# penincillin/IHMR

Measured on AMD Instinct MI355X. Metric: images/sec, IHMR-OPT 200-iter refinement batch=64 (ms/refine-iter: latency.ms_per_refine_iter; amortised: ms_per_refine_iter_amortised), higher is better.
Workload: dtype f32

## Files before the change

### ihmr_amd/csrc/ihmr_hip.hip

```cpp
#include <math.h>
#include <stdio.h>
#include <stdlib.h>
#include <string.h>

#include <algorithm>
#include <atomic>
#include <mutex>
#include <vector>

#include "ihmr_common.h"
#include "mano_lbs.h"
#include "sdf_collision.h"
#include "preprocess.h"
#include "augment.h"
#include "render.h"
#include "mlp_infer.h"
#include "refine.h"
#include "encoder.h"
#include "encoder_bf16.h"
#include "evaluate.h"
#include "train.h"
#include "train_conv.h"
#include "copy_pack.h"
#include "launch_plan.h"
// ... 111 lines not shown
        for (int k = 0; k < 3; ++k) {
            const int32_t id = h->faces[(f < NF ? f : 0) * 3 + k];
            if (id < 0 || id >= NV) { delete m; return -1; }
            fsoa[(size_t)k * NFP + f] = id;
        }
    std::vector<uint32_t> fpk(NFP, 0u);
    for (int f = 0; f < NFP; ++f)
        fpk[f] = (uint32_t)fsoa[f] | ((uint32_t)fsoa[(size_t)NFP + f] << 10) | ((uint32_t)fsoa[(size_t)2 * NFP + f] << 20);
    std::vector<float> pd4, sd4, vt4;
    pack4(pd.data(), NPF, pd4);
    pack4(sd_t.data(), 10, sd4);
    pack4(vt.data(), 1, vt4);
    int rc = 0;
    rc |= upload_as(&m->pd4, pd4); rc |= upload_as(&m->sd4, sd4); rc |= upload_as(&m->vt4, vt4);
    rc |= upload(&m->v_template, vt); rc |= upload(&m->shapedirs_t, sd_t); rc |= upload(&m->posedirs, pd);
    rc |= upload(&m->J_template, J_t); rc |= upload(&m->J_shapedirs, J_sd); rc |= upload(&m->weights, wts);
    rc |= upload_as(&m->w4_w, w4w); rc |= upload(&m->w4_j, w4j);
    m->sparse4 = sparse4;
    rc |= upload(&m->pose_mean, pm); rc |= upload(&m->parents, par); rc |= upload(&m->depth, depth);
    rc |= upload(&m->tip_ids, tips); rc |= upload(&m->wj_start, start); rc |= upload(&m->wj_vert, wv);
    rc |= upload(&m->wj_w, ww); rc |= upload(&m->seg_q, seg_q); rc |= upload(&m->jseg_start, jseg); rc |= upload(&m->faces, fsoa); rc |= upload(&m->faces_pk, fpk); rc |= upload(&m->J_regressor, jr);
    m->max_depth = maxd;
    m->nnz = (int)wv.size();
    m->nseg = (int)seg_q.size() - 1;
    if (m->nseg > LBS_SEG_CAP) { ihmr_mano_destroy(m); return -1; }
    {
        const int dyn = m->nseg * 12 * (int)sizeof(float);
        hipError_t e1 = hipFuncSetAttribute((const void*)lbs_bwd1_kernel<true>, hipFuncAttributeMaxDynamicSharedMemorySize, dyn);
        hipError_t e2 = hipFuncSetAttribute((const void*)lbs_bwd1_kernel<false>, hipFuncAttributeMaxDynamicSharedMemorySize, dyn);
        if (e1 != hipSuccess || e2 != hipSuccess) { ihmr_mano_destroy(m); return (int)(e1 != hipSuccess ? e1 : e2); }
        int dev = 0, lds_max = 0;
        (void)hipGetDevice(&dev);
        (void)hipDeviceGetAttribute(&lds_max, hipDeviceAttributeMaxSharedMemoryPerBlock, dev);
        const void* tails[3] = {(const void*)opt_tail_kernel<true, true>, (const void*)opt_tail_kernel<true>, (const void*)opt_tail_kernel<false>};
        m->tail_fits = 1;
        const int tail_dyn = opt_tail_dynamic_lds(m->nseg);
        for (const void* k : tails) {
            hipFuncAttributes fa;
            if (hipFuncGetAttributes(&fa, k) != hipSuccess || (long)fa.sharedSizeBytes + tail_dyn > (long)lds_max ||
                hipFuncSetAttribute(k, hipFuncAttributeMaxDynamicSharedMemorySize, tail_dyn) != hipSuccess)
                m->tail_fits = 0;
        }
        (void)hipGetLastError();
    }
    if (rc) return rc;
    *out = m;
    return 0;
}

extern "C" int ihmr_mano_destroy(ihmr_mano* m) {
    if (!m) return 0;
    void* ptrs[] = {m->v_template, m->shapedirs_t, m->posedirs, m->J_template, m->J_shapedirs, m->weights, m->pose_mean,
                    m->parents, m->depth, m->tip_ids, m->wj_start, m->wj_vert, m->wj_w, m->faces, m->J_regressor, m->pd4, m->sd4, m->vt4, m->seg_q, m->jseg_start,
                    m->w4_w, m->w4_j, m->faces_pk};
    for (void* p : ptrs)
        if (p) (void)hipFree(p);
    delete m;
    return 0;
}

extern "C" int ihmr_mano_update_shapedirs(ihmr_mano* m, const float* shapedirs_host) {
    if (!m || !shapedirs_host) return -1;
    std::vector<float> jr((size_t)NJ * NV), vt(NV3), sd_t, J_t, J_sd;
    HIP_TRY(hipMemcpy(jr.data(), m->J_regressor, jr.size() * 4, hipMemcpyDeviceToHost));
    HIP_TRY(hipMemcpy(vt.data(), m->v_template, vt.size() * 4, hipMemcpyDeviceToHost));
    derive_shape_constants(jr.data(), vt.data(), shapedirs_host, sd_t, J_t, J_sd);
    HIP_TRY(hipMemcpy(m->shapedirs_t, sd_t.data(), sd_t.size() * 4, hipMemcpyHostToDevice));
    HIP_TRY(hipMemcpy(m->J_shapedirs, J_sd.data(), J_sd.size() * 4, hipMemcpyHostToDevice));
    std::vector<float> sd4;
    pack4(sd_t.data(), 10, sd4);
    HIP_TRY(hipMemcpy(m->sd4, sd4.data(), sd4.size() * 4, hipMemcpyHostToDevice));
    return 0;
}

extern "C" size_t ihmr_mano_workspace_bytes(int N) { return lbs_ws_bytes(N); }

template <bool TWO_HAND, int MODE>
static void lbs_skin_launch_mode(const ihmr_mano* m, int N, int B, float* verts, float* joints, const LbsWork& wk, float* pose_off, hipStream_t st) {
    const bool small = N <= LBS_SMALL_MAX_HANDS;
    const int hg8 = 8 * (small ? LBS_HG_SMALL : LBS_HG);
    const dim3 skin_grid(8, 4 * ((N + hg8 - 1) / hg8));
    if (small) hipLaunchKernelGGL((lbs_skin_kernel<TWO_HAND, MODE, LBS_HG_SMALL>), skin_grid, dim3(LBS_THREADS), 0, st, *m, (const float*)wk.skel, N, B,
                                  verts, joints, wk.v_posed, pose_off);
    else hipLaunchKernelGGL((lbs_skin_kernel<TWO_HAND, MODE, LBS_HG>), skin_grid, dim3(LBS_THREADS), 0, st, *m, (const float*)wk.skel, N, B, verts,
                            joints, wk.v_posed, pose_off);
}
#define LBS_SKIN_FULL 0
#define LBS_SKIN_REUSE 1
#define LBS_SKIN_KEEP_P 2
#define LBS_SKIN_FULL_STORE_P 3
static int g_force_full_skin = 0;
template <bool TWO_HAND>
static void lbs_skin_launch(const ihmr_mano* m, int mode, int N, int B, float* verts, float* joints, const LbsWork& wk, hipStream_t st) {
    if (g_force_full_skin && (mode == LBS_SKIN_KEEP_P || mode == LBS_SKIN_FULL_STORE_P)) mode = LBS_SKIN_FULL;
    if (mode == LBS_SKIN_REUSE) lbs_skin_launch_mode<TWO_HAND, LBS_MODE_REUSE>(m, N, B, verts, joints, wk, nullptr, st);
    else if (mode == LBS_SKIN_KEEP_P) lbs_skin_launch_mode<TWO_HAND, LBS_MODE_KEEP_P>(m, N, B, verts, joints, wk, wk.pose_off, st);
    else lbs_skin_launch_mode<TWO_HAND, LBS_MODE_FULL>(m, N, B, verts, joints, wk, mode == LBS_SKIN_FULL_STORE_P ? wk.pose_off : nullptr, st);
}
extern "C" int ihmr_debug_force_full_skin(int force) {
    const int prev = g_force_full_skin;
    g_force_full_skin = force ? 1 : 0;
    return prev;
}

static void lbs_forward_launch(const ihmr_mano* m, bool two_hand, const float* orient, const float* pose, const float* betas,
                               const float* trans, int N, int B, float* verts, float* joints, const LbsWork& wk, hipStream_t st) {
    if (two_hand) {
        hipLaunchKernelGGL(lbs_skel_kernel<true>, dim3(N), dim3(192), 0, st, *m, orient, pose, betas, trans, B, wk.skel, joints);
        lbs_skin_launch<true>(m, LBS_SKIN_FULL, N, B, verts, joints, wk, st);
    } else {
        hipLaunchKernelGGL(lbs_skel_kernel<false>, dim3(N), dim3(192), 0, st, *m, orient, pose, betas, trans, B, wk.skel, joints);
        lbs_skin_launch<false>(m, LBS_SKIN_FULL, N, B, verts, joints, wk, st);
    }
}

static int g_bwd2_streaming = 0;
extern "C" int ihmr_debug_force_lbs_bwd2_streaming(int force) {
    const int prev = g_bwd2_streaming;
    g_bwd2_streaming = force ? 1 : 0;
    return prev;
}

static void lbs_backward_launch(const ihmr_mano* m, bool two_hand, int N, int B, const float* d_verts, const float* d_joints,
                                float* d_orient, float* d_pose, float* d_betas, float* d_trans, int need_mask, const LbsWork& wk,
                                hipStream_t st, bool bwd1_done = false) {
    const size_t part_lds = (size_t)m->nseg * 12 * sizeof(float);
    if (bwd1_done) {}
    else if (two_hand)
        hipLaunchKernelGGL(lbs_bwd1_kernel<true>, dim3(N), dim3(LBS_THREADS), part_lds, st, *m, wk, B, d_verts, d_joints, d_orient,
                           d_betas, d_trans, need_mask);
    else
        hipLaunchKernelGGL(lbs_bwd1_kernel<false>, dim3(N), dim3(LBS_THREADS), part_lds, st, *m, wk, B, d_verts, d_joints, d_orient,
                           d_betas, d_trans, need_mask);
    if (need_mask & 2) {
// ... 166 lines not shown
extern "C" int ihmr_opt_forward_losses(const ihmr_mano* m, const ihmr_mano* m_left, const ihmr_opt_io* io, int B,
                                       const ihmr_opt_weights* w, void* stream) {
    if (!m || !io || !w || B <= 0 || 2 * B > SDF_MAX_HANDS) return -1;
    hipStream_t st = (hipStream_t)stream;
    OptWork wk = opt_carve(io->workspace, B);
    int rc = opt_forward(m, m_left, io, wk, B, *w, kNoStep, st);
    if (rc) return rc;
    return (int)hipGetLastError();
}

extern "C" int ihmr_opt_run_stage(const ihmr_mano* m, const ihmr_mano* m_left, const ihmr_opt_io* io, int B,
                                  const ihmr_opt_weights* w, const ihmr_opt_stage* sg, void* stream) {
    if (!m || !io || !w || !sg || B <= 0 || 2 * B > SDF_MAX_HANDS || sg->n_iters <= 0 || sg->save_freq <= 0) return -1;
    if (sg->param_mask <= 0 || sg->param_mask > 255 || sg->select_loss < 0 || sg->select_loss > 2) return -1;
    if (sg->optimizer != IHMR_OPTIM_ADAM && sg->optimizer != IHMR_OPTIM_SGD) return -1;
    hipStream_t st = (hipStream_t)stream;
    OptWork wk = opt_carve(io->workspace, B);
    const int pm = sg->param_mask;
    const int need_mask = ((pm & (IHMR_PB_ORIENT_R | IHMR_PB_ORIENT_L)) ? 1 : 0) | ((pm & (IHMR_PB_POSE_R | IHMR_PB_POSE_L)) ? 2 : 0) |
                          ((pm & (IHMR_PB_SHAPE_R | IHMR_PB_SHAPE_L)) ? 4 : 0) | ((pm & IHMR_PB_TRANS) ? 8 : 0);
    const int need_cam = (pm & IHMR_PB_CAM) ? 1 : 0, sgd = sg->optimizer == IHMR_OPTIM_SGD;
    int S = 0;
    ParamStep step{0, 0.f, 0.f, 1.f, -1, 1, 0};
    const bool vposed_fixed = (pm & (IHMR_PB_POSE_R | IHMR_PB_POSE_L | IHMR_PB_SHAPE_R | IHMR_PB_SHAPE_L)) == 0;
    const bool pose_fixed = (pm & (IHMR_PB_POSE_R | IHMR_PB_POSE_L)) == 0;
    const int keep_mode = vposed_fixed ? LBS_SKIN_REUSE : (pose_fixed ? LBS_SKIN_KEEP_P : LBS_SKIN_FULL);
    const int first_mode = (!vposed_fixed && pose_fixed) ? LBS_SKIN_FULL_STORE_P : LBS_SKIN_FULL;
    const bool fused_tail = need_mask != 0 && !io->no_fused_tail && m->tail_fits;
    int static_mask = ((pm & (IHMR_PB_ORIENT_R | IHMR_PB_POSE_R | IHMR_PB_SHAPE_R)) ? 0 : 1) |
                      ((pm & (IHMR_PB_ORIENT_L | IHMR_PB_POSE_L | IHMR_PB_SHAPE_L | IHMR_PB_TRANS | IHMR_PB_SHAPE_R)) ? 0 : 2);
    if ((pm & IHMR_PB_TRANS) && !(pm & (IHMR_PB_ORIENT_L | IHMR_PB_POSE_L | IHMR_PB_SHAPE_L | IHMR_PB_SHAPE_R)) && io->sdf_no_static_reuse == 0)
        static_mask |= 2 | (2 << 2);
    const bool pose_stage = (need_mask & 2) != 0;
    const size_t tail_lds = (size_t)opt_tail_dynamic_lds(m->nseg);
    const int lists_first = sg->keep_lists ? 3 : 2;
    for (int it = 0; it < sg->n_iters; ++it) {
        const double t = (double)(it + 1);
        const double bc1 = 1.0 - pow(0.9, t), bc2 = 1.0 - pow(0.999, t);
        const ParamStep next{pm, w->shape_reg, sgd ? sg->lr : (float)((double)sg->lr / bc1), (float)sqrt(bc2),
                             (it % sg->save_freq == 0) ? S++ : -1, 0, sgd};
        if (fused_tail) {
            int rc = opt_forward(m, m_left, io, wk, B, *w, step, st, need_cam, it == 0 ? first_mode : (vposed_fixed ? -1 : keep_mode), it == 0 ? lists_first : 1,
                                 it == 0 || pose_stage, false, static_mask);
            if (rc) return rc;
            SdfWorkspace ws = opt_sdf_ws(io, wk, B, it == 0 ? lists_first : 1, static_mask);
            VertLayout vl{io->verts, (long)NV3, (long)B * NV3};
            hipEvent_t tcur;
            const bool timed = g_timer != nullptr;
            if (timed) { if (int rc2 = timed_begin(&tcur, st)) return rc2; }
            const TailArgs ta{*m, *io, wk, B, *w, vl, ws, need_cam, need_mask, next, ws.inside_count};
            if (vposed_fixed && it + 1 < sg->n_iters)
                hipLaunchKernelGGL((opt_tail_kernel<true, true>), dim3(B), dim3(SDF_SAMPLE_THREADS), tail_lds, st, ta);
            else if (!pose_stage && it + 1 < sg->n_iters)
                hipLaunchKernelGGL(opt_tail_kernel<true>, dim3(B), dim3(SDF_SAMPLE_THREADS), tail_lds, st, ta);
            else
                hipLaunchKernelGGL(opt_tail_kernel<false>, dim3(B), dim3(SDF_SAMPLE_THREADS), tail_lds, st, ta);
            if (timed) { if (int rc2 = timed_next(&tcur, IHMR_TIMED_OPT_TAIL, st)) return rc2; (void)hipEventDestroy(tcur); }
            if (pose_stage)
                lbs_backward_launch(m, true, 2 * B, B, wk.g_verts, wk.g_joints, wk.g_orient, wk.g_pose, wk.g_shape, wk.g_trans, need_mask,
                                    wk.lbs, st, true);
        } else {
            int rc = opt_forward(m, m_left, io, wk, B, *w, step, st, need_cam, it == 0 ? first_mode : keep_mode, it == 0 ? lists_first : 1, true, true, static_mask);
            if (rc) return rc;
            if (need_mask)
                lbs_backward_launch(m, true, 2 * B, B, wk.g_verts, wk.g_joints, wk.g_orient, wk.g_pose, wk.g_shape, wk.g_trans, need_mask,
                                    wk.lbs, st);
        }
        step = next;
    }
    hipLaunchKernelGGL(opt_adam_kernel, dim3(B), dim3(128), 0, st, *io, wk, B, step);
    hipLaunchKernelGGL(opt_select_kernel, dim3((B + 63) / 64), dim3(64), 0, st, *io, B, S, *sg);
    return (int)hipGetLastError();
}

extern "C" int ihmr_opt_set_params(const ihmr_opt_io* io, const float* final_params, int B, void* stream) {
    if (!io || !final_params || B <= 0) return -1;
    hipLaunchKernelGGL(opt_unpack_params_kernel, dim3(B), dim3(128), 0, (hipStream_t)stream, *io, final_params, B);
    return (int)hipGetLastError();
}

extern "C" size_t ihmr_mlp_workspace_bytes(int B) { return ((size_t)B * (512 + 256 + 128 + 126) * sizeof(float) + 256 + 255) & ~(size_t)255; }
static float* mlp_acc_joints(void* workspace, int B) { return (float*)((char*)workspace + 256) + (size_t)B * (512 + 256 + 128); }

static int mlp_fill_select(MlpSelect& s, const ihmr_mlp_tables* t, const ihmr_mlp_stage* stage, int mode, void* workspace) {
// ... 721 lines not shown
```

### ihmr_amd/csrc/mano_lbs.h

```cpp
#pragma once
#include "ihmr_common.h"

#define LBS_THREADS 256
#define LBS_HG 8
#define LBS_HG_SMALL 4
#define LBS_SMALL_MAX_HANDS 256
#define LBS_TILE_V 195
#define LBS_KG 25
#define LBS_KC 3
#define LBS_SEG 13
#define LBS_SEG_CAP 1024
#define LBS_CSR_CAP 4096

#define SK_R 0
#define SK_J 144
#define SK_G 192
#define SK_A 384
#define SK_PF 576
#define SK_POSE 712
#define SK_BETA 760
#define SK_SHIFT 770
#define SK_STRIDE 784

struct LbsWork {
    float* skel;
    float* v_posed;
    float* dvp;
    float* chain;
    float* dpf_part;
    float* pose_off;
};

static inline size_t lbs_ws_bytes(int N) {
    size_t n = (size_t)N * (SK_STRIDE + 3 * NV3 + 192 + LBS_KG * 136) * sizeof(float);
    return ((n + 255) & ~(size_t)255) + 6 * 256;
}

static inline LbsWork lbs_carve(void* ws, int N) {
    LbsWork w;
    char* p = (char*)ws;
    auto take = [&](size_t bytes) { char* r = p; p += (bytes + 255) & ~(size_t)255; return (float*)r; };
    w.skel = take((size_t)N * SK_STRIDE * 4);
    w.v_posed = take((size_t)N * NV3 * 4);
    w.dvp = take((size_t)N * NV3 * 4);
    w.chain = take((size_t)N * 192 * 4);
    w.dpf_part = take((size_t)LBS_KG * N * 136 * 4);
    w.pose_off = take((size_t)N * NV3 * 4);
    return w;
}

template <bool TWO_HAND>
__device__ __forceinline__ void lbs_skel_hand(const ihmr_mano& m, const float* __restrict__ orient,
                                              const float* __restrict__ pose, const float* __restrict__ betas,
                                              const float* __restrict__ trans, int B, float* __restrict__ skel,
                                              float* __restrict__ joints, float* sk, int h, int tid_in, bool active = true) {
    const bool left = TWO_HAND && h >= B;
    const int tid = active ? tid_in : (1 << 20);
    float* sR = sk + SK_R; float* sJ = sk + SK_J; float* sG = sk + SK_G; float* sA = sk + SK_A;
    const int my_depth = active ? m.depth[tid_in / 12] : -1, my_parent = active ? m.parents[tid_in / 12] : 0;
    float* sPF = sk + SK_PF; float* sPose = sk + SK_POSE; float* sBeta = sk + SK_BETA; float* sShift = sk + SK_SHIFT;
    if (tid < 48) {
        float v = tid < 3 ? orient[h * 3 + tid] : pose[h * 45 + tid - 3];
        if (left && (tid % 3) != 0) v = -v;
        sPose[tid] = v + m.pose_mean[tid];
    }
    if (tid >= 64 && tid < 74) sBeta[tid - 64] = betas[h * 10 + tid - 64];
    if (tid >= 128 && tid < 142) sk[SK_SHIFT + tid - 128] = 0.f;
    if (tid == 150) sPF[135] = 0.f;
    __syncthreads();
    if (tid < NJ) rodrigues_fwd(&sPose[3 * tid], &sR[9 * tid]);
    if (tid >= 64 && tid < 64 + 48) {
        const int e = tid - 64;
        float acc = m.J_template[e];
#pragma unroll
        for (int l = 0; l < 10; ++l) acc = __builtin_fmaf(m.J_shapedirs[e * 10 + l], sBeta[l], acc);
        sJ[e] = acc;
    }
    __syncthreads();
    if (tid < NPF) {
        const int j = 1 + tid / 9, e = tid % 9;
        sPF[tid] = sR[9 * j + e] - ((e == 0 || e == 4 || e == 8) ? 1.0f : 0.0f);
    }
    if (tid >= 160 && tid < 172) {
        const int e = tid - 160, r = e / 4, c = e % 4;
        sG[e] = c < 3 ? sR[3 * r + c] : sJ[r];
    }
    if (TWO_HAND && left && tid >= 176 && tid < 179) {
        const int k = tid - 176;
        const float* br = betas + (h - B) * 10;
        float jr = m.J_template[k];
#pragma unroll
        for (int l = 0; l < 10; ++l) jr = __builtin_fmaf(m.J_shapedirs[k * 10 + l], br[l], jr);
        const float jl = k == 0 ? -sJ[0] : sJ[k];
        sShift[k] = trans[(h - B) * 3 + k] + (jr - jl);
    }
    __syncthreads();
    for (int d = 1; d <= m.max_depth; ++d) {
        const int j = tid / 12, e = tid % 12, r = e / 4, c = e % 4;
        if (my_depth == d) {
            const int p = my_parent;
            sG[12 * j + e] = lbs_chain_elem(sG + 12 * p, sR + 9 * j, sJ + 3 * j, sJ + 3 * p, r, c);
        }
        __syncthreads();
    }
    if (active) {
        const int j = tid / 12, e = tid % 12, r = e / 4, c = e % 4;
        sA[12 * j + e] = lbs_rel_elem(sG + 12 * j, sJ + 3 * j, r, c);
    }
    __syncthreads();
    for (int i = tid; i < SK_STRIDE; i += 192) skel[(size_t)h * SK_STRIDE + i] = sk[i];
    if (tid < NJ * 3) {
        const int j = tid / 3, k = tid % 3;
// ... 881 lines not shown
```

### ihmr_amd/csrc/refine.h

```cpp
#pragma once
#include "ihmr_common.h"

#define LOSS_THREADS 64
#define OPT_NPARAM IHMR_OPT_NPARAM

struct OptWork {
    LbsWork lbs;
    float* joints_raw;
    float* g_verts;
    float* g_joints;
    float* g_trans_direct;
    float* g_cam;
    float* g_orient;
    float* g_pose;
    float* g_shape;
    float* g_trans;
    void* sdf_ws;
};

static inline size_t opt_ws_bytes(int B) {
    size_t n = 0;
    n += (size_t)2 * B * NV3 * 4;
    n += lbs_ws_bytes(2 * B);
    n += (size_t)B * 42 * 3 * 4 * 2;
    n += (size_t)B * (3 + 6 + 90 + 20 + 3 + 3 + 1) * 4;
    n = (n + 255) & ~(size_t)255;
    n += 8192;
    return n + sdf_ws_bytes(2 * B, true);
}

static inline OptWork opt_carve(void* ws, int B) {
    OptWork w;
    char* p = (char*)ws;
    auto take = [&](size_t bytes) { char* r = p; p += (bytes + 255) & ~(size_t)255; return r; };
    w.lbs = lbs_carve(take(lbs_ws_bytes(2 * B)), 2 * B);
    w.g_verts = (float*)take((size_t)2 * B * NV3 * 4);
    w.joints_raw = (float*)take((size_t)B * 42 * 3 * 4);
    w.g_joints = (float*)take((size_t)B * 42 * 3 * 4);
    w.g_trans_direct = (float*)take((size_t)B * 3 * 4);
    w.g_orient = (float*)take((size_t)B * 6 * 4);
    w.g_pose = (float*)take((size_t)B * 90 * 4);
    w.g_shape = (float*)take((size_t)B * 20 * 4);
    w.g_trans = (float*)take((size_t)B * 3 * 4);
    w.g_cam = (float*)take((size_t)B * 3 * 4);
    w.sdf_ws = (void*)p;
    return w;
}

__constant__ int c_finger_ids[20] = {1, 2, 3, 17, 4, 5, 6, 18, 7, 8, 9, 20, 10, 11, 12, 19, 13, 14, 15, 16};

struct LossShared {
    float raw[42][3], p1[42][3], p2[42][3], g2[42][3], acc[8][LOSS_THREADS], gsum[2][3];
};
#define LOSS_SYNC()                                                  \
    do {                                                             \
        __builtin_amdgcn_fence(__ATOMIC_RELEASE, "workgroup");       \
        __builtin_amdgcn_wave_barrier();                             \
        __builtin_amdgcn_fence(__ATOMIC_ACQUIRE, "workgroup");       \
    } while (0)

__device__ __forceinline__ void opt_loss_wave(const ihmr_opt_io& io, const OptWork& wk, int B, const ihmr_opt_weights& w,
                                              LossShared& sh, int b, int j, int need_cam, LbsBwdShared* gj_lds = nullptr) {
    const bool act = j < 42;
    const int Bn = io.norm_batch > 0 ? io.norm_batch : B;
    const int jj = act ? j : 0;
    const float cs = io.cam[b * 3], ctx = io.cam[b * 3 + 1], cty = io.cam[b * 3 + 2];
    float r[3], t2[3], tg2[3], tg3[4], ti3[4];
#pragma unroll
    for (int k = 0; k < 3; ++k) {
        r[k] = wk.joints_raw[(b * 42 + jj) * 3 + k];
        t2[k] = io.init_joints_2d[(b * 42 + jj) * 3 + k];
        tg2[k] = io.gt_joints_2d[(b * 42 + jj) * 3 + k];
    }
#pragma unroll
    for (int k = 0; k < 4; ++k) { tg3[k] = io.gt_joints_3d[(b * 42 + jj) * 4 + k]; ti3[k] = io.init_joints_3d[(b * 42 + jj) * 4 + k]; }
    float tp4[4] = {0.f, 0.f, 0.f, 0.f}, tgt4[4] = {0.f, 0.f, 0.f, 0.f}, tr3[3] = {0.f, 0.f, 0.f};
    if (j == 5) {
#pragma unroll
        for (int k = 0; k < 4; ++k) { tp4[k] = io.init_hand_trans_j[b * 4 + k]; tgt4[k] = io.gt_hand_trans[b * 4 + k]; }
#pragma unroll
        for (int k = 0; k < 3; ++k) tr3[k] = io.trans[b * 3 + k];
    }
    __builtin_amdgcn_sched_barrier(0);
    if (act) {
#pragma unroll
        for (int k = 0; k < 3; ++k) sh.raw[j][k] = r[k];
    }
    LOSS_SYNC();

    float l2d_p = 0.f, l2d_gt = 0.f, g_raw[3] = {0.f, 0.f, 0.f};
    if (act) {
        const float px = (r[0] + ctx) * cs, py = (r[1] + cty) * cs;
        io.joints_2d[(b * 42 + j) * 2] = px;
        io.joints_2d[(b * 42 + j) * 2 + 1] = py;
        const float dx = t2[0] - px, dy = t2[1] - py;
// ... 214 lines not shown
}
__device__ __forceinline__ void opt_snapshot_losses(const ihmr_opt_io& io, int B, const ParamStep& st, int b, int e) {
    if (st.snap_idx >= 0 && e < 3) io.snap_loss[((size_t)st.snap_idx * 3 + e) * B + b] = io.loss_batch[e * B + b];
}

__global__ __launch_bounds__(128) void opt_adam_kernel(ihmr_opt_io io, OptWork wk, int B, ParamStep st) {
    opt_snapshot_losses(io, B, st, blockIdx.x, threadIdx.x);
    if ((int)threadIdx.x < OPT_NPARAM) opt_param_apply(io, wk, B, st, blockIdx.x, threadIdx.x);
}

__global__ __launch_bounds__(384) void opt_adam_skel_kernel(ihmr_mano m, ihmr_opt_io io, OptWork wk, int B, ParamStep st,
                                                            int* inside_count) {
    TL_SCOPE(7);
    __shared__ float sk[2][SK_STRIDE];
    const int b = blockIdx.x, tid = threadIdx.x;
    if (b == 0 && tid >= 192 && tid < 192 + SDF_NZERO) sdf_zero_counter(inside_count, tid - 192);
    if (st.reset_state && tid < OPT_NPARAM) { io.adam_m[b * OPT_NPARAM + tid] = 0.f; io.adam_v[b * OPT_NPARAM + tid] = 0.f; }
    if (st.mask && tid < OPT_NPARAM) { opt_snapshot_losses(io, B, st, b, tid); opt_param_apply(io, wk, B, st, b, tid); }
    __syncthreads();
    const int hl = tid / 192;
    lbs_skel_hand<true>(m, io.orient, io.pose, io.shape, io.trans, B, wk.lbs.skel, wk.joints_raw, sk[hl], hl * B + b, tid % 192);
}

#ifdef TAIL_STAMPS
__device__ long long g_tail_stamps[3][4096][8];
#define TAIL_TK(k) do { if (threadIdx.x == 0) { const long long now_ = (long long)__builtin_readcyclecounter(); if (blockIdx.x < 4096) g_tail_stamps[STEP + SKIN][blockIdx.x][k] += now_ - tk_prev_; tk_prev_ = now_; } } while (0)
#else
#define TAIL_TK(k)
#endif
static inline int opt_tail_dynamic_lds(int nseg) { return 2 * nseg * 12 * (int)sizeof(float); }
struct TailArgs {
    ihmr_mano m; ihmr_opt_io io; OptWork wk; int B; ihmr_opt_weights w; VertLayout vl; SdfWorkspace ws; int need_cam, need_mask;
    ParamStep st; int* inside_count;
};
__device__ __forceinline__ const TailArgs& tail_args() {
    typedef const __attribute__((address_space(4))) TailArgs* ArgPtr;
    ArgPtr p = (ArgPtr)__builtin_amdgcn_kernarg_segment_ptr();
    asm volatile("" : "+s"(p));
    return *(const TailArgs*)p;
}
template <bool STEP, bool SKIN = false>
__global__ __launch_bounds__(SDF_SAMPLE_THREADS, 4) void opt_tail_kernel(TailArgs) {
    TL_SCOPE(3 + (STEP ? 1 : 0) + (SKIN ? 1 : 0));
    __shared__ LossShared sh;
    __shared__ float red16[SDF_SAMPLE_THREADS / WAVE];
    __shared__ LbsBwdShared bw[2];
    extern __shared__ __attribute__((aligned(16))) float tail_part[];
    const int b = blockIdx.x, tid = threadIdx.x;
#ifdef TAIL_STAMPS
    long long tk_prev_ = (long long)__builtin_readcyclecounter();
    if (tid == 0 && blockIdx.x < 4096) g_tail_stamps[STEP + SKIN][blockIdx.x][7] += 1;
#endif
    const int hl = tid / LBS_THREADS;
    {
    const TailArgs& a = tail_args();
    const int B = a.B, need_mask = a.need_mask;
    const ihmr_opt_io io = a.io; const OptWork wk = a.wk; const ihmr_opt_weights w = a.w; const SdfWorkspace ws = a.ws;
    const VertLayout vl = a.vl;
    if ((need_mask & 7) != 0) {
        lds_dma_dwords(wk.lbs.v_posed + (size_t)(hl * B + b) * NV3, bw[hl].vp, NV3, tid % LBS_THREADS, LBS_THREADS);
        lds_dma_dwords(wk.lbs.skel + (size_t)(hl * B + b) * SK_STRIDE, bw[hl].sk, SK_STRIDE, tid % LBS_THREADS, LBS_THREADS);
    } else if (SKIN) {
        lds_dma_dwords(wk.lbs.skel + (size_t)(hl * B + b) * SK_STRIDE, bw[hl].sk, SK_STRIDE, tid % LBS_THREADS, LBS_THREADS);
    }
    const float mask = (io.hand_type_array[b * 2] + io.hand_type_array[b * 2 + 1]) > 1.5f ? 1.f : 0.f;
    const float gs = w.collision * mask / (ws.loss_div * (float)(io.norm_batch > 0 ? io.norm_batch : B));
// ... 35 lines not shown
    uint32_t jr[VR];
    if (SKIN) {
#pragma unroll
        for (int r = 0; r < VR; ++r) {
            const int v = min(lt + r * LBS_THREADS, NV - 1);
            const float* s0 = wk.lbs.v_posed + ((size_t)hv * NV + v) * 3;
            vp[r][0] = s0[0]; vp[r][1] = s0[1]; vp[r][2] = s0[2];
            wr[r] = m.sparse4 ? m.w4_w[v] : make_float4(0.f, 0.f, 0.f, 0.f);
            jr[r] = m.sparse4 ? m.w4_j[v] : 0u;
        }
        __builtin_amdgcn_sched_barrier(0);
    }
    if (SKIN && (need_mask & 7) == 0) {
        if (tid < 3) {
            const float* br = io.shape + (size_t)b * 10;
            float jr = m.J_template[tid];
#pragma unroll
            for (int l = 0; l < 10; ++l) jr = __builtin_fmaf(m.J_shapedirs[tid * 10 + l], br[l], jr);
            const float* sJl = bw[1].sk + SK_J;
            const float jl = tid == 0 ? -sJl[0] : sJl[tid];
            const float sh = io.trans[b * 3 + tid] + (jr - jl);
            bw[1].sk[SK_SHIFT + tid] = sh;
            wk.lbs.skel[((size_t)B + b) * SK_STRIDE + SK_SHIFT + tid] = sh;
        }
        __syncthreads();
        if (tid < NJ * 3) {
            const int j = tid / 3, k = tid % 3;
            const float val = bw[1].sk[SK_G + 12 * j + 4 * k + 3];
            wk.joints_raw[((size_t)b * 42 + 21 + j) * 3 + k] = (k == 0 ? -val : val) + bw[1].sk[SK_SHIFT + k];
        }
    } else {
        const int hs = tid / 192;
        lbs_skel_hand<true>(m, io.orient, io.pose, io.shape, io.trans, B, wk.lbs.skel, wk.joints_raw, bw[hs < 2 ? hs : 0].sk, (hs < 2 ? hs : 0) * B + b, tid % 192,
                            hs < 2);
    }
    TAIL_TK(3);
    if (!SKIN) return;
    const float* sA = bw[hl].sk + SK_A;
    const float* sShift = bw[hl].sk + SK_SHIFT;
#pragma unroll
    for (int r = 0; r < VR; ++r) {
        const int v = lt + r * LBS_THREADS;
        if (v >= NV) break;
        float T[12];
#pragma unroll
        for (int e = 0; e < 12; ++e) T[e] = 0.f;
        if (m.sparse4) {
            const float wv[4] = {wr[r].x, wr[r].y, wr[r].z, wr[r].w};
#pragma unroll
            for (int sI = 0; sI < 4; ++sI) {
                const float4* A4 = reinterpret_cast<const float4*>(sA + 12 * (int)((jr[r] >> (8 * sI)) & 0xffu));
#pragma unroll
                for (int q = 0; q < 3; ++q) {
                    const float4 a = A4[q];
                    T[4 * q] = __builtin_fmaf(wv[sI], a.x, T[4 * q]);
                    T[4 * q + 1] = __builtin_fmaf(wv[sI], a.y, T[4 * q + 1]);
                    T[4 * q + 2] = __builtin_fmaf(wv[sI], a.z, T[4 * q + 2]);
                    T[4 * q + 3] = __builtin_fmaf(wv[sI], a.w, T[4 * q + 3]);
                }
            }
        } else {
            for (int j = 0; j < NJ; ++j) {
                const float wj = m.weights[v * NJ + j];
#pragma unroll
                for (int e = 0; e < 12; ++e) T[e] = __builtin_fmaf(wj, sA[12 * j + e], T[e]);
            }
        }
        float out[3];
#pragma unroll
        for (int q = 0; q < 3; ++q) out[q] = T[4 * q + 0] * vp[r][0] + T[4 * q + 1] * vp[r][1] + T[4 * q + 2] * vp[r][2] + T[4 * q + 3];
        if (hl == 1) {
            out[0] = -out[0] + sShift[0];
            out[1] = out[1] + sShift[1];
            out[2] = out[2] + sShift[2];
        }
        float* dst = io.verts + ((size_t)hv * NV + v) * 3;
        dst[0] = out[0]; dst[1] = out[1]; dst[2] = out[2];
#pragma unroll
        for (int t = 0; t < IHMR_NUM_TIPS; ++t)
            if (v == m.tip_ids[t]) {
                float* jd = wk.joints_raw + ((size_t)b * 42 + (hl ? 21 : 0) + NJ + t) * 3;
                jd[0] = out[0]; jd[1] = out[1]; jd[2] = out[2];
            }
    }
    TAIL_TK(4);
}

__global__ __launch_bounds__(256) void mlp_camera_select_kernel(ihmr_opt_io io, OptWork wk, int B, ihmr_opt_weights w, MlpSelect sel) {
    __shared__ LossShared sh;
    const int b = blockIdx.x, tid = threadIdx.x;
    if (tid < WAVE) {
        opt_loss_wave(io, wk, B, w, sh, b, tid, 0);
        if (tid == 0) io.loss_batch[(size_t)2 * B + b] = sel.prev_loss[(size_t)sel.idx[b] * 3 + 2];
    }
    mlp_select_sample(sel, io.loss_batch, B, b);
}

__global__ __launch_bounds__(128) void opt_unpack_params_kernel(ihmr_opt_io io, const float* __restrict__ packed, int B) {
    const int b = blockIdx.x, e = threadIdx.x;
    if (e >= 122) return;
    const float v = packed[(size_t)b * 122 + e];
    if (e < 3) io.cam[b * 3 + e] = v;
    else if (e < 6) io.orient[(size_t)b * 3 + (e - 3)] = v;
    else if (e < 51) io.pose[(size_t)b * 45 + (e - 6)] = v;
    else if (e < 54) io.orient[((size_t)B + b) * 3 + (e - 51)] = v;
    else if (e < 99) io.pose[((size_t)B + b) * 45 + (e - 54)] = v;
    else if (e < 109) io.shape[(size_t)b * 10 + (e - 99)] = v;
    else if (e < 119) io.shape[((size_t)B + b) * 10 + (e - 109)] = v;
    else io.trans[b * 3 + (e - 119)] = v;
}

__global__ void opt_select_kernel(ihmr_opt_io io, int B, int S, ihmr_opt_stage sg) {
    const int b = blockIdx.x * blockDim.x + threadIdx.x;
    if (b >= B) return;
    float bar[3];
#pragma unroll
    for (int l = 0; l < 3; ++l) bar[l] = io.snap_loss[(size_t)l * B + b] * sg.filter_factor[l];
    int best = 0;
// ... 16 lines not shown
```

### ihmr_amd/hip.py

```python
from __future__ import annotations

import ctypes as C
import os
import os.path as osp
import subprocess

import numpy as np
import torch

_HERE = osp.dirname(osp.abspath(__file__))
LIB_PATH = osp.join(_HERE, "libihmr_hip.so")
SRC_DIR = osp.join(_HERE, "csrc")
HIPCC_FLAGS = ["--offload-arch=gfx950", "-O3", "-std=c++17", "-ffp-contract=off", "-shared", "-fPIC"]

NUM_VERTS, NUM_FACES, NUM_JOINTS, OPT_NPARAM = 778, 1538, 16, 122
PARAM_BLOCKS = dict(pred_cam_params=(1, 0, 3), pred_hand_trans=(2, 3, 3), pred_right_orient=(4, 6, 3), pred_left_orient=(8, 9, 3),
                    pred_right_pose_params=(16, 12, 45), pred_left_pose_params=(32, 57, 45),
                    pred_right_shape_params=(64, 102, 10), pred_left_shape_params=(128, 112, 10))
LOSS_IDS = dict(joints_2d_loss_p=0, joints_3d_loss_p=1, collision_loss=2)
OPTIMIZERS = dict(adam=0, sgd=1)

EXPORTED_SYMBOLS = [
    "ihmr_mano_create", "ihmr_mano_destroy", "ihmr_mano_update_shapedirs", "ihmr_mano_workspace_bytes", "ihmr_mano_lbs_fwd",
    "ihmr_mano_lbs_bwd",
    "ihmr_sdf_workspace_bytes", "ihmr_sdf_collision", "ihmr_sdf_collision_ex", "ihmr_sdf_dense_grid", "ihmr_opt_workspace_bytes",
    "ihmr_opt_run_stage", "ihmr_opt_forward_losses", "ihmr_opt_sdf_stats", "ihmr_opt_sdf_counters", "ihmr_opt_sdf_inside_bits", "ihmr_opt_stage_graph_create",
    "ihmr_opt_forward_graph_create", "ihmr_graph_launch", "ihmr_graph_destroy", "ihmr_opt_set_params", "ihmr_eval_metrics", "ihmr_eval_mpvpe", "ihmr_conv_igemm", "ihmr_maxpool3x3s2",
    "ihmr_avgpool_relu", "ihmr_preprocess_images", "ihmr_mlp_train_grad", "ihmr_transpose", "ihmr_relu_backward", "ihmr_colsum",
    "ihmr_adam_step", "ihmr_bn_workspace_bytes", "ihmr_bn_train_forward", "ihmr_bn_train_backward", "ihmr_conv_wgrad",
    "ihmr_dilate2", "ihmr_interleave2", "ihmr_pack_dgrad_weight", "ihmr_maxpool3x3s2_backward", "ihmr_avgpool_relu_backward", "ihmr_set_kernel_timer", "ihmr_flush_kernel_timer",
    "ihmr_mlp_workspace_bytes", "ihmr_mlp_stage_head", "ihmr_mlp_forward_select", "ihmr_mlp_camera_select", "ihmr_opt_forward_verts",
    "ihmr_debug_force_lbs_bwd2_streaming", "ihmr_debug_force_full_skin", "ihmr_version", "ihmr_copy_segments", "ihmr_root_align_joints",
    "ihmr_augment_images", "ihmr_augment_labels",
    "ihmr_render_workspace_bytes", "ihmr_render_meshes", "ihmr_draw_keypoints",
    "ihmr_conv_igemm_bf16", "ihmr_pack_image_bf16", "ihmr_maxpool3x3s2_bf16", "ihmr_avgpool_relu_bf16", "ihmr_cast_f32_bf16",
]


class ManoArrays(C.Structure):
    _fields_ = [(n, C.c_void_p) for n in ("v_template", "shapedirs", "posedirs", "J_regressor", "lbs_weights", "parents",
                                          "hands_mean", "faces", "tip_ids")]


class OptIO(C.Structure):
    _fields_ = [(n, C.c_void_p) for n in (
        "cam", "trans", "orient", "pose", "shape",
        "init_joints_2d", "init_joints_3d", "init_hand_trans_j", "gt_joints_2d", "gt_joints_3d", "gt_hand_trans",
        "hand_type_array",
        "verts", "joints_3d", "joints_2d", "loss_batch", "coll_per_vert", "coll_origin_scale",
        "snap_params", "snap_loss", "selected", "adam_m", "adam_v", "workspace")] + [
        ("norm_batch", C.c_int), ("sdf_align_corners", C.c_int), ("sdf_loss_divisor", C.c_float), ("sdf_swap_xz", C.c_int),
        ("sdf_no_candidate_lists", C.c_int), ("sdf_no_static_reuse", C.c_int),
        ("no_fused_tail", C.c_int)]


class CopySeg(C.Structure):
    _fields_ = [("src", C.c_void_p), ("dst", C.c_void_p), ("rows", C.c_int), ("width", C.c_int), ("src_ld", C.c_int), ("dst_ld", C.c_int)]


COPY_MAX_SEGS = 32


def copy_segments(pairs):
    segs = []
    for src, dst in pairs:
# ... 285 lines not shown
```

### include/ihmr_hip.h

```cpp
#ifndef IHMR_HIP_H
#define IHMR_HIP_H

#include <stddef.h>
#include <stdint.h>

#ifdef __cplusplus
extern "C" {
#endif

#define IHMR_NUM_VERTS 778
#define IHMR_NUM_FACES 1538
#define IHMR_NUM_JOINTS 16
#define IHMR_NUM_TIPS 5
#define IHMR_SDF_GRID 32

typedef struct ihmr_mano_arrays {
    const float* v_template;
    const float* shapedirs;
    const float* posedirs;
    const float* J_regressor;
    const float* lbs_weights;
    const int32_t* parents;
    const float* hands_mean;
    const int32_t* faces;
// ... 195 lines not shown
int ihmr_draw_keypoints(uint8_t* img, const float* kps, const float* weight, const uint8_t* colour, int B, int S, int K, void* stream);

#define IHMR_TIMED_SDF_PREP 0
#define IHMR_TIMED_SDF_DIST 1
#define IHMR_TIMED_OPT_TAIL 2
#define IHMR_TIMED_KERNELS 4
typedef struct ihmr_kernel_timer { double ms[IHMR_TIMED_KERNELS]; long n[IHMR_TIMED_KERNELS]; double ms_event_pair; long n_event_pair; } ihmr_kernel_timer;
int ihmr_set_kernel_timer(ihmr_kernel_timer* t);
int ihmr_flush_kernel_timer(void);

typedef struct ihmr_mlp_net { const float* w[4]; const float* b[4]; int ldw[4]; int k_out; int col[122]; } ihmr_mlp_net;
typedef struct ihmr_mlp_tables {
    const int64_t* idx;
    uint8_t* data_idxs_all;
    float* img_feat_all;
    float* prev_final;
    float* prev_loss;
    const float* img_feat;
    float* new_params;
    float* final_params;
    uint8_t* kept;
} ihmr_mlp_tables;
typedef struct ihmr_mlp_stage { int n_filter; int filter_loss[4]; float filter_factor[4]; int select_loss; } ihmr_mlp_stage;
size_t ihmr_mlp_workspace_bytes(int B);
int ihmr_mlp_stage_head(const ihmr_mlp_net* net, const ihmr_mlp_tables* t, const ihmr_opt_io* io, int B, void* workspace, void* stream);
int ihmr_mlp_forward_select(const ihmr_mano* m, const ihmr_mano* m_left, const ihmr_opt_io* io, int B, const ihmr_opt_weights* w,
                            const ihmr_mlp_tables* t, const ihmr_mlp_stage* stage, int mode, void* workspace, void* stream);
int ihmr_mlp_camera_select(const ihmr_opt_io* io, int B, const ihmr_opt_weights* w, const ihmr_mlp_tables* t, const ihmr_mlp_stage* stage,
                           void* workspace, void* stream);
int ihmr_opt_forward_verts(const ihmr_mano* m, const ihmr_opt_io* io, int B, void* stream);

int ihmr_debug_force_lbs_bwd2_streaming(int force);
int ihmr_debug_force_full_skin(int force);

const char* ihmr_version(void);

#ifdef __cplusplus
}
#endif
#endif
```

Before: 29030.

## Add translation-only fused tail kernel and skip rotation recompute for fixed hands

Adds a dedicated opt_tail_kernel_trans for stages where only translation is optimized. It computes the trans gradient as a direct sum of per-vertex SDF gradients and caches the skinned left-hand vertices once, so later iterations only add the shift instead of redoing skinning. It also passes a keep_rot flag so the skeleton pass skips the Rodrigues and pose-feature recompute for hands whose orient and pose are frozen. The cost is an extra per-batch vertex buffer in the workspace and correctness that depends on the cached state staying valid across iterations.

```diff
diff --git a/ihmr_amd/csrc/ihmr_hip.hip b/ihmr_amd/csrc/ihmr_hip.hip
--- a/ihmr_amd/csrc/ihmr_hip.hip
+++ b/ihmr_amd/csrc/ihmr_hip.hip
@@ -167,13 +167,15 @@
         int dev = 0, lds_max = 0;
         (void)hipGetDevice(&dev);
         (void)hipDeviceGetAttribute(&lds_max, hipDeviceAttributeMaxSharedMemoryPerBlock, dev);
-        const void* tails[3] = {(const void*)opt_tail_kernel<true, true>, (const void*)opt_tail_kernel<true>, (const void*)opt_tail_kernel<false>};
+        const void* tails[4] = {(const void*)opt_tail_kernel<true, true>, (const void*)opt_tail_kernel<true>, (const void*)opt_tail_kernel<false>,
+                                (const void*)opt_tail_kernel_trans};
         m->tail_fits = 1;
         const int tail_dyn = opt_tail_dynamic_lds(m->nseg);
         for (const void* k : tails) {
             hipFuncAttributes fa;
-            if (hipFuncGetAttributes(&fa, k) != hipSuccess || (long)fa.sharedSizeBytes + tail_dyn > (long)lds_max ||
-                hipFuncSetAttribute(k, hipFuncAttributeMaxDynamicSharedMemorySize, tail_dyn) != hipSuccess)
+            const int dyn_k = k == (const void*)opt_tail_kernel_trans ? 0 : tail_dyn;
+            if (hipFuncGetAttributes(&fa, k) != hipSuccess || (long)fa.sharedSizeBytes + dyn_k > (long)lds_max ||
+                (dyn_k && hipFuncSetAttribute(k, hipFuncAttributeMaxDynamicSharedMemorySize, dyn_k) != hipSuccess))
                 m->tail_fits = 0;
         }
         (void)hipGetLastError();
@@ -235,6 +237,12 @@
 extern "C" int ihmr_debug_force_full_skin(int force) {
     const int prev = g_force_full_skin;
     g_force_full_skin = force ? 1 : 0;
+    return prev;
+}
+static int g_force_generic_tail = 0;
+extern "C" int ihmr_debug_force_generic_tail(int force) {
+    const int prev = g_force_generic_tail;
+    g_force_generic_tail = force ? 1 : 0;
     return prev;
 }
 
@@ -467,6 +475,9 @@
     if ((pm & IHMR_PB_TRANS) && !(pm & (IHMR_PB_ORIENT_L | IHMR_PB_POSE_L | IHMR_PB_SHAPE_L | IHMR_PB_SHAPE_R)) && io->sdf_no_static_reuse == 0)
         static_mask |= 2 | (2 << 2);
     const bool pose_stage = (need_mask & 2) != 0;
+    const bool trans_tail = vposed_fixed && need_mask == 8 && !g_force_generic_tail;
+    const int keep_rot = ((need_mask & 7) == 0 || g_force_generic_tail) ? 0
+                         : (((pm & (IHMR_PB_ORIENT_R | IHMR_PB_POSE_R)) ? 0 : 1) | ((pm & (IHMR_PB_ORIENT_L | IHMR_PB_POSE_L)) ? 0 : 2));
     const size_t tail_lds = (size_t)opt_tail_dynamic_lds(m->nseg);
     const int lists_first = sg->keep_lists ? 3 : 2;
     for (int it = 0; it < sg->n_iters; ++it) {
@@ -483,8 +494,10 @@
             hipEvent_t tcur;
             const bool timed = g_timer != nullptr;
             if (timed) { if (int rc2 = timed_begin(&tcur, st)) return rc2; }
-            const TailArgs ta{*m, *io, wk, B, *w, vl, ws, need_cam, need_mask, next, ws.inside_count};
-            if (vposed_fixed && it + 1 < sg->n_iters)
+            const TailArgs ta{*m, *io, wk, B, *w, vl, ws, need_cam, need_mask, next, ws.inside_count, keep_rot, it == 0 ? 1 : 0};
+            if (trans_tail && it + 1 < sg->n_iters)
+                hipLaunchKernelGGL(opt_tail_kernel_trans, dim3(B), dim3(SDF_SAMPLE_THREADS), 0, st, ta);
+            else if (vposed_fixed && it + 1 < sg->n_iters)
                 hipLaunchKernelGGL((opt_tail_kernel<true, true>), dim3(B), dim3(SDF_SAMPLE_THREADS), tail_lds, st, ta);
             else if (!pose_stage && it + 1 < sg->n_iters)
                 hipLaunchKernelGGL(opt_tail_kernel<true>, dim3(B), dim3(SDF_SAMPLE_THREADS), tail_lds, st, ta);
diff --git a/ihmr_amd/csrc/mano_lbs.h b/ihmr_amd/csrc/mano_lbs.h
--- a/ihmr_amd/csrc/mano_lbs.h
+++ b/ihmr_amd/csrc/mano_lbs.h
@@ -53,22 +53,23 @@
 __device__ __forceinline__ void lbs_skel_hand(const ihmr_mano& m, const float* __restrict__ orient,
                                               const float* __restrict__ pose, const float* __restrict__ betas,
                                               const float* __restrict__ trans, int B, float* __restrict__ skel,
-                                              float* __restrict__ joints, float* sk, int h, int tid_in, bool active = true) {
+                                              float* __restrict__ joints, float* sk, int h, int tid_in, bool active = true,
+                                              bool keep_rot = false) {
     const bool left = TWO_HAND && h >= B;
     const int tid = active ? tid_in : (1 << 20);
     float* sR = sk + SK_R; float* sJ = sk + SK_J; float* sG = sk + SK_G; float* sA = sk + SK_A;
     const int my_depth = active ? m.depth[tid_in / 12] : -1, my_parent = active ? m.parents[tid_in / 12] : 0;
     float* sPF = sk + SK_PF; float* sPose = sk + SK_POSE; float* sBeta = sk + SK_BETA; float* sShift = sk + SK_SHIFT;
-    if (tid < 48) {
+    if (!keep_rot && tid < 48) {
         float v = tid < 3 ? orient[h * 3 + tid] : pose[h * 45 + tid - 3];
         if (left && (tid % 3) != 0) v = -v;
         sPose[tid] = v + m.pose_mean[tid];
     }
     if (tid >= 64 && tid < 74) sBeta[tid - 64] = betas[h * 10 + tid - 64];
     if (tid >= 128 && tid < 142) sk[SK_SHIFT + tid - 128] = 0.f;
-    if (tid == 150) sPF[135] = 0.f;
-    __syncthreads();
-    if (tid < NJ) rodrigues_fwd(&sPose[3 * tid], &sR[9 * tid]);
+    if (!keep_rot && tid == 150) sPF[135] = 0.f;
+    __syncthreads();
+    if (!keep_rot && tid < NJ) rodrigues_fwd(&sPose[3 * tid], &sR[9 * tid]);
     if (tid >= 64 && tid < 64 + 48) {
         const int e = tid - 64;
         float acc = m.J_template[e];
@@ -77,7 +78,7 @@
         sJ[e] = acc;
     }
     __syncthreads();
-    if (tid < NPF) {
+    if (!keep_rot && tid < NPF) {
         const int j = 1 + tid / 9, e = tid % 9;
         sPF[tid] = sR[9 * j + e] - ((e == 0 || e == 4 || e == 8) ? 1.0f : 0.0f);
     }
diff --git a/ihmr_amd/csrc/refine.h b/ihmr_amd/csrc/refine.h
--- a/ihmr_amd/csrc/refine.h
+++ b/ihmr_amd/csrc/refine.h
@@ -15,6 +15,7 @@
     float* g_pose;
     float* g_shape;
     float* g_trans;
+    float* kept_left;
     void* sdf_ws;
 };
 
@@ -24,6 +25,7 @@
     n += lbs_ws_bytes(2 * B);
     n += (size_t)B * 42 * 3 * 4 * 2;
     n += (size_t)B * (3 + 6 + 90 + 20 + 3 + 3 + 1) * 4;
+    n += (size_t)B * NV3 * 4 + 256;
     n = (n + 255) & ~(size_t)255;
     n += 8192;
     return n + sdf_ws_bytes(2 * B, true);
@@ -43,6 +45,7 @@
     w.g_shape = (float*)take((size_t)B * 20 * 4);
     w.g_trans = (float*)take((size_t)B * 3 * 4);
     w.g_cam = (float*)take((size_t)B * 3 * 4);
+    w.kept_left = (float*)take((size_t)B * NV3 * 4);
     w.sdf_ws = (void*)p;
     return w;
 }
@@ -59,8 +62,9 @@
         __builtin_amdgcn_fence(__ATOMIC_ACQUIRE, "workgroup");       \
     } while (0)
 
+template <class GJ = LbsBwdShared>
 __device__ __forceinline__ void opt_loss_wave(const ihmr_opt_io& io, const OptWork& wk, int B, const ihmr_opt_weights& w,
-                                              LossShared& sh, int b, int j, int need_cam, LbsBwdShared* gj_lds = nullptr) {
+                                              LossShared& sh, int b, int j, int need_cam, GJ* gj_lds = nullptr) {
     const bool act = j < 42;
     const int Bn = io.norm_batch > 0 ? io.norm_batch : B;
     const int jj = act ? j : 0;
@@ -341,6 +345,8 @@
 struct TailArgs {
     ihmr_mano m; ihmr_opt_io io; OptWork wk; int B; ihmr_opt_weights w; VertLayout vl; SdfWorkspace ws; int need_cam, need_mask;
     ParamStep st; int* inside_count;
+    int keep_rot;
+    int fill_kept;
 };
 __device__ __forceinline__ const TailArgs& tail_args() {
     typedef const __attribute__((address_space(4))) TailArgs* ArgPtr;
@@ -442,7 +448,7 @@
     } else {
         const int hs = tid / 192;
         lbs_skel_hand<true>(m, io.orient, io.pose, io.shape, io.trans, B, wk.lbs.skel, wk.joints_raw, bw[hs < 2 ? hs : 0].sk, (hs < 2 ? hs : 0) * B + b, tid % 192,
-                            hs < 2);
+                            hs < 2, ((a.keep_rot >> (hs < 2 ? hs : 0)) & 1) != 0);
     }
     TAIL_TK(3);
     if (!SKIN) return;
@@ -494,6 +500,155 @@
             }
     }
     TAIL_TK(4);
+}
+
+struct TransTailHand { float g[NV3]; float gj[21][3]; };
+__global__ __launch_bounds__(SDF_SAMPLE_THREADS, 4) void opt_tail_kernel_trans(TailArgs) {
+    TL_SCOPE(5);
+    __shared__ LossShared sh;
+    __shared__ float red16[SDF_SAMPLE_THREADS / WAVE];
+    __shared__ TransTailHand th[2];
+    __shared__ __attribute__((aligned(16))) float skl[SK_STRIDE];
+    __shared__ float wsum[LBS_THREADS / WAVE][4];
+    const int b = blockIdx.x, tid = threadIdx.x;
+    {
+    const TailArgs& a = tail_args();
+    const int B = a.B;
+    const ihmr_opt_io io = a.io; const OptWork wk = a.wk; const ihmr_opt_weights w = a.w; const SdfWorkspace ws = a.ws;
+    const VertLayout vl = a.vl;
+    lds_dma_dwords(wk.lbs.skel + ((size_t)B + b) * SK_STRIDE, skl, SK_STRIDE, tid, SDF_SAMPLE_THREADS);
+    const float mask = (io.hand_type_array[b * 2] + io.hand_type_array[b * 2 + 1]) > 1.5f ? 1.f : 0.f;
+    const float gs = w.collision * mask / (ws.loss_div * (float)(io.norm_batch > 0 ? io.norm_batch : B));
+    if (tid >= OPT_SAMPLE_WORKERS) {
+        opt_loss_wave(io, wk, B, w, sh, b, tid - OPT_SAMPLE_WORKERS, a.need_cam, th);
+        if (tid == OPT_SAMPLE_WORKERS) red16[OPT_SAMPLE_WORKERS / WAVE] = 0.f;
+        __syncthreads();
+    } else {
+        sdf_sample_cells(vl, ws, io.loss_batch + 2 * B, B, io.hand_type_array, red16, b, OPT_SAMPLE_WORKERS, SdfEmitTail{gs, th[0].g, th[1].g});
+    }
+    }
+    asm volatile("s_waitcnt vmcnt(0)" ::: "memory");
+    __syncthreads();
+    constexpr int VR = (NV + LBS_THREADS - 1) / LBS_THREADS;
+    if (tid < LBS_THREADS) {
+        float s0 = 0.f, s1 = 0.f, s2 = 0.f;
+#pragma unroll
+        for (int r = 0; r < VR; ++r) {
+            const int v = tid + r * LBS_THREADS;
+            s0 += v < NV ? -th[1].g[3 * v] : 0.f;
+            s1 += v < NV ? th[1].g[3 * v + 1] : 0.f;
+            s2 += v < NV ? th[1].g[3 * v + 2] : 0.f;
+        }
+        float gjl[3] = {0.f, 0.f, 0.f};
+        if (tid < 21) { gjl[0] = -th[1].gj[tid][0]; gjl[1] = th[1].gj[tid][1]; gjl[2] = th[1].gj[tid][2]; }
+        s0 += gjl[0]; s1 += gjl[1]; s2 += gjl[2];
+        s0 = wave_reduce_sum_dpp(s0); s1 = wave_reduce_sum_dpp(s1); s2 = wave_reduce_sum_dpp(s2);
+        if (tid % WAVE == 0) { wsum[tid / WAVE][0] = s0; wsum[tid / WAVE][1] = s1; wsum[tid / WAVE][2] = s2; }
+    }
+    __syncthreads();
+    if (tid < 3) {
+        float t = 0.f;
+#pragma unroll
+        for (int wv = 0; wv < LBS_THREADS / WAVE; ++wv) t += wsum[wv][tid];
+        tail_args().wk.g_trans[b * 3 + tid] = t;
+    }
+    __syncthreads();
+    constexpr int ER = (NV3 + SDF_SAMPLE_THREADS - 1) / SDF_SAMPLE_THREADS;
+    float kept[ER], kept_tip = 0.f;
+#pragma unroll
+    for (int r = 0; r < ER; ++r) kept[r] = 0.f;
+    {
+    const TailArgs& a = tail_args();
+    const ihmr_opt_io io = a.io; const OptWork wk = a.wk; const ParamStep st = a.st;
+    if (!a.fill_kept) {
+#pragma unroll
+        for (int r = 0; r < ER; ++r) kept[r] = wk.kept_left[(size_t)b * NV3 + min(tid + r * SDF_SAMPLE_THREADS, NV3 - 1)];
+        if (tid < IHMR_NUM_TIPS * 3) kept_tip = wk.kept_left[(size_t)b * NV3 + 3 * a.m.tip_ids[tid / 3] + tid % 3];
+    }
+    if (b == 0 && tid >= 384 && tid < 384 + SDF_NZERO) sdf_zero_counter(a.inside_count, tid - 384);
+    if (st.mask && tid < OPT_NPARAM) { opt_snapshot_losses(io, a.B, st, b, tid); opt_param_apply(io, wk, a.B, st, b, tid); }
+    }
+    __syncthreads();
+    const TailArgs& a = tail_args();
+    const int B = a.B;
+    const ihmr_mano m = a.m; const ihmr_opt_io io = a.io; const OptWork wk = a.wk;
+    if (tid < 3) {
+        const float* br = io.shape + (size_t)b * 10;
+        float jr = m.J_template[tid];
+#pragma unroll
+        for (int l = 0; l < 10; ++l) jr = __builtin_fmaf(m.J_shapedirs[tid * 10 + l], br[l], jr);
+        const float* sJl = skl + SK_J;
+        const float jl = tid == 0 ? -sJl[0] : sJl[tid];
+        const float sh = io.trans[b * 3 + tid] + (jr - jl);
+        skl[SK_SHIFT + tid] = sh;
+        wk.lbs.skel[((size_t)B + b) * SK_STRIDE + SK_SHIFT + tid] = sh;
+    }
+    __syncthreads();
+    if (tid < NJ * 3) {
+        const int j = tid / 3, k = tid % 3;
+        const float val = skl[SK_G + 12 * j + 4 * k + 3];
+        wk.joints_raw[((size_t)b * 42 + 21 + j) * 3 + k] = (k == 0 ? -val : val) + skl[SK_SHIFT + k];
+    }
+    const float* sShift = skl + SK_SHIFT;
+    float* dstv = io.verts + ((size_t)B + b) * NV3;
+    if (a.fill_kept) {
+        const float* sA = skl + SK_A;
+#pragma unroll 1
+        for (int v = tid; v < NV; v += SDF_SAMPLE_THREADS) {
+            const float* s0 = wk.lbs.v_posed + ((size_t)(B + b) * NV + v) * 3;
+            const float vp[3] = {s0[0], s0[1], s0[2]};
+            float T[12];
+#pragma unroll
+            for (int e = 0; e < 12; ++e) T[e] = 0.f;
+            if (m.sparse4) {
+                const float4 wr = m.w4_w[v];
+                const uint32_t jr = m.w4_j[v];
+                const float wv[4] = {wr.x, wr.y, wr.z, wr.w};
+#pragma unroll
+                for (int sI = 0; sI < 4; ++sI) {
+                    const float4* A4 = reinterpret_cast<const float4*>(sA + 12 * (int)((jr >> (8 * sI)) & 0xffu));
+#pragma unroll
+                    for (int q = 0; q < 3; ++q) {
+                        const float4 a4 = A4[q];
+                        T[4 * q] = __builtin_fmaf(wv[sI], a4.x, T[4 * q]);
+                        T[4 * q + 1] = __builtin_fmaf(wv[sI], a4.y, T[4 * q + 1]);
+                        T[4 * q + 2] = __builtin_fmaf(wv[sI], a4.z, T[4 * q + 2]);
+                        T[4 * q + 3] = __builtin_fmaf(wv[sI], a4.w, T[4 * q + 3]);
+                    }
+                }
+            } else {
+#pragma unroll 1
+                for (int j = 0; j < NJ; ++j) {
+                    const float wj = m.weights[v * NJ + j];
+#pragma unroll
+                    for (int e = 0; e < 12; ++e) T[e] = __builtin_fmaf(wj, sA[12 * j + e], T[e]);
+                }
+            }
+            float out[3];
+#pragma unroll
+            for (int q = 0; q < 3; ++q) out[q] = T[4 * q + 0] * vp[0] + T[4 * q + 1] * vp[1] + T[4 * q + 2] * vp[2] + T[4 * q + 3];
+            out[0] = -out[0];
+            float* kd = wk.kept_left + (size_t)b * NV3 + 3 * v;
+            kd[0] = out[0]; kd[1] = out[1]; kd[2] = out[2];
+#pragma unroll
+            for (int q = 0; q < 3; ++q) out[q] = out[q] + sShift[q];
+            dstv[3 * v] = out[0]; dstv[3 * v + 1] = out[1]; dstv[3 * v + 2] = out[2];
+#pragma unroll
+            for (int t = 0; t < IHMR_NUM_TIPS; ++t)
+                if (v == m.tip_ids[t]) {
+                    float* jd = wk.joints_raw + ((size_t)b * 42 + 21 + NJ + t) * 3;
+                    jd[0] = out[0]; jd[1] = out[1]; jd[2] = out[2];
+                }
+        }
+        return;
+    }
+#pragma unroll
+    for (int r = 0; r < ER; ++r) {
+        const int i = tid + r * SDF_SAMPLE_THREADS;
+        if (i < NV3) dstv[i] = kept[r] + sShift[i % 3];
+    }
+    if (tid < IHMR_NUM_TIPS * 3)
+        wk.joints_raw[((size_t)b * 42 + 21 + NJ + tid / 3) * 3 + tid % 3] = kept_tip + sShift[tid % 3];
 }
 
 __global__ __launch_bounds__(256) void mlp_camera_select_kernel(ihmr_opt_io io, OptWork wk, int B, ihmr_opt_weights w, MlpSelect sel) {
diff --git a/ihmr_amd/hip.py b/ihmr_amd/hip.py
--- a/ihmr_amd/hip.py
+++ b/ihmr_amd/hip.py
@@ -30,7 +30,7 @@
     "ihmr_adam_step", "ihmr_bn_workspace_bytes", "ihmr_bn_train_forward", "ihmr_bn_train_backward", "ihmr_conv_wgrad",
     "ihmr_dilate2", "ihmr_interleave2", "ihmr_pack_dgrad_weight", "ihmr_maxpool3x3s2_backward", "ihmr_avgpool_relu_backward", "ihmr_set_kernel_timer", "ihmr_flush_kernel_timer",
     "ihmr_mlp_workspace_bytes", "ihmr_mlp_stage_head", "ihmr_mlp_forward_select", "ihmr_mlp_camera_select", "ihmr_opt_forward_verts",
-    "ihmr_debug_force_lbs_bwd2_streaming", "ihmr_debug_force_full_skin", "ihmr_version", "ihmr_copy_segments", "ihmr_root_align_joints",
+    "ihmr_debug_force_lbs_bwd2_streaming", "ihmr_debug_force_full_skin", "ihmr_debug_force_generic_tail", "ihmr_version", "ihmr_copy_segments", "ihmr_root_align_joints",
     "ihmr_augment_images", "ihmr_augment_labels",
     "ihmr_render_workspace_bytes", "ihmr_render_meshes", "ihmr_draw_keypoints",
     "ihmr_conv_igemm_bf16", "ihmr_pack_image_bf16", "ihmr_maxpool3x3s2_bf16", "ihmr_avgpool_relu_bf16", "ihmr_cast_f32_bf16",
diff --git a/include/ihmr_hip.h b/include/ihmr_hip.h
--- a/include/ihmr_hip.h
+++ b/include/ihmr_hip.h
@@ -251,6 +251,7 @@
 
 int ihmr_debug_force_lbs_bwd2_streaming(int force);
 int ihmr_debug_force_full_skin(int force);
+int ihmr_debug_force_generic_tail(int force);
 
 const char* ihmr_version(void);
 
```

Result: faster. 29760 (median of 6 runs) (+2.5%).
